# meringlab/FlashWeave.jl

Measured on AMD Instinct MI355X. Metric: ci_tests_per_sec, higher is better.
Workload: dtype f64

## Files before the change

### flashweave.jl_amd/csrc/fw_devhiton.hip

```cpp
#include <algorithm>
#include <cassert>
#include <cstring>
#include <condition_variable>
#include <mutex>
#include <thread>
#include <vector>

#include "fw_internal.h"
#define MI_MAX_K FW_MAX_K_FAST
#include "fw_mi_core.h"
#include "fw_fz_core.h"
#include "fw_unrank.h"

namespace {

struct DhTgt {
    int32_t T, phase, pos, nc;
    int32_t na, ntpc, npc, wl_n;
    long long co;
    long long cand_off;
    long long wl_off, nb_off;
    int32_t nb_n, cap;
    int32_t jactive, nsp;
    int32_t cur, pad0;
// ... 2026 lines not shown
        run += dh_ceil_div(win[act[t]], seglen, inv) + (sp[act[t]] ? dh_ceil_div(win2[act[t]], seglen, inv) * sp[act[t]] : 0u);
    }
    if (tid == 0) {
        seg0[na] = (long long)ns;
        g->ns = ns;
        g->any_big = 0u;
        g->seglen = (unsigned int)seglen;
        g->launched_ranks = total;
        g->n_live_prev = n_live;
        if (n_live == 0u) g->done = 1u;
        const unsigned int r = g->rounds;
        g->ns_ring[r & 63u] = ns;
        g->rounds = r + 1u;
        if (log && r < log_cap) log[r] = make_ulonglong2(total, ((unsigned long long)n_live << 32) | ns);
    }
}

__global__ __launch_bounds__(1024) void dh_plan_kernel(int ntg, DhGlobal *__restrict__ g, const unsigned long long *__restrict__ win,
                                                       const unsigned int *__restrict__ sp, const unsigned long long *__restrict__ win2,
                                                       const int32_t *__restrict__ act_all, long long *__restrict__ seg0, DhPlanArgs PA)
{
    dh_plan_dev<1024>(ntg, g, win, sp, win2, act_all, seg0, PA);
}
__global__ __launch_bounds__(256) void dh_plan_small_kernel(int ntg, DhGlobal *__restrict__ g, const unsigned long long *__restrict__ win,
                                                            const unsigned int *__restrict__ sp, const unsigned long long *__restrict__ win2,
                                                            const int32_t *__restrict__ act_all, long long *__restrict__ seg0, DhPlanArgs PA)
{
    dh_plan_dev<256>(ntg, g, win, sp, win2, act_all, seg0, PA);
}

__global__ __launch_bounds__(256) void dh_tmat_build_kernel(const DhTgt *__restrict__ tg, int ntg, const int32_t *__restrict__ nb_idx,
                                                            const float *__restrict__ cor, int p, float *__restrict__ tmat)
{
    __shared__ int32_t s_id[4096];
    const DhTgt &x = tg[blockIdx.x];
    if (x.tm_off < 0) return;
    const int m = x.nb_n + 1;
    const int32_t *ids = nb_idx + x.nb_off;
    for (int b = threadIdx.x; b < m; b += 256) s_id[b] = b == 0 ? x.T : ids[b - 1];
    __syncthreads();
    float *M = tmat + x.tm_off;
    for (int a0 = (int)blockIdx.y * 4; a0 < m; a0 += (int)gridDim.y * 4)
        for (int b = threadIdx.x; b < m; b += 256) {
            const size_t col = (size_t)s_id[b];
            float v[4];
#pragma unroll
            for (int q = 0; q < 4; ++q) v[q] = a0 + q < m ? cor[(size_t)s_id[a0 + q] * (size_t)p + col] : 0.0f;
#pragma unroll
            for (int q = 0; q < 4; ++q)
                if (a0 + q < m) M[(size_t)(a0 + q) * m + b] = v[q];
        }
}

__device__ __forceinline__ void dh_fill_one(const unsigned int s, const DhTgt *__restrict__ tg, int ntg, DhGlobal *__restrict__ g,
                                            const long long *__restrict__ seg0, const DhArrays &A, FwSeg *__restrict__ segs, int d1,
                                            const int32_t *__restrict__ act)
{
    int lo = 0, hi = (int)g->n_act;
    while (lo < hi) {
        const int mid = (lo + hi) >> 1;
        if (seg0[mid] <= (long long)s)
            lo = mid + 1;
        else
            hi = mid;
    }
    const DhTgt &x = tg[act[(size_t)g->act_sel * ntg + lo - 1]];
    const unsigned long long seglen = g->seglen;
    unsigned long long k = (unsigned long long)((long long)s - seg0[lo - 1]);
    const int32_t *cands = x.phase == 0 ? A.cand0 + x.cand_off : A.tpc_key + x.co;
    unsigned int slot = 0;
    if (x.nsp > 0) {
        const unsigned int all = (unsigned int)(seg0[lo] - seg0[lo - 1]);
        const unsigned int n0 = x.spmode == 1 ? dh_ceil_div(x.jwin, seglen, 1.0 / (double)seglen) : all / (1u + (unsigned int)x.nsp);
        if ((unsigned int)k >= n0) {
            const unsigned int per = (all - n0) / (unsigned int)x.nsp;
            slot = 1u + ((unsigned int)k - n0) / per;
            k -= (unsigned long long)n0 + (unsigned long long)(slot - 1u) * per;
        }
    }
    const bool acc_mode = slot > 0u && x.spmode == 1;
    FwSeg sg;
    sg.X = x.T;
    sg.Y = cands[x.pos + (int)slot];
    sg.acc_off = DH_ACC_OFF(x, x.phase == 1 ? (x.cur + (int)slot) % d1 : x.cur, d1);
    sg.acc_len = x.na + (acc_mode ? 1 : 0);
    if (sg.acc_len > FW_TAB_A) g->any_big = 1u;
    sg.pad = act[(size_t)g->act_sel * ntg + lo - 1];
    const unsigned long long lo_r = acc_mode ? 0ull : x.jnext;
    sg.start = lo_r + k * seglen;
    const unsigned long long hi_r = lo_r + (slot > 0u ? x.jwin2 : x.jwin);
    sg.end = sg.start + seglen < hi_r ? sg.start + seglen : hi_r;
    const bool has_tm = A.tmat != nullptr && x.tm_off >= 0;
    sg.tm = has_tm ? (uint64_t)(A.tmat + x.tm_off) : 0ull;
    sg.tm_ids = has_tm ? (uint64_t)(A.nb_idx + x.nb_off) : 0ull;
    sg.tm_m = has_tm ? x.nb_n + 1 : 0;
    sg.pad1 = 0;
    segs[s] = sg;
}
__global__ __launch_bounds__(256) void dh_fill_kernel(const DhTgt *__restrict__ tg, int ntg, DhGlobal *__restrict__ g,
                                                      const long long *__restrict__ seg0, const DhArrays A,
                                                      FwSeg *__restrict__ segs, int d1, const int32_t *__restrict__ act)
{
    const unsigned int s = blockIdx.x * 256 + threadIdx.x;
    if (s >= g->ns) return;
    dh_fill_one(s, tg, ntg, g, seg0, A, segs, d1, act);
}


__global__ __launch_bounds__(1024) void dh_compact_kernel(const DhTgt *__restrict__ tg, int ntg, DhGlobal *__restrict__ g,
                                                          int32_t *__restrict__ act_all)
{
    __shared__ unsigned int s_wsum[16];
    const int tid = threadIdx.x, lane = tid & 63, wave = tid >> 6;
    const int na = (int)g->n_act;
    const unsigned int sel = g->act_sel;
    const int32_t *src = act_all + (size_t)sel * ntg;
    int32_t *dst = act_all + (size_t)(sel ^ 1u) * ntg;
    const int per = (na + 1023) / 1024;
    const int b = tid * per, e = (b + per) < na ? (b + per) : na;
    unsigned int local = 0u;
    for (int i = b; i < e; ++i) {
        const DhTgt &x = tg[src[i]];
        local += (x.phase != 2 || x.jactive) ? 1u : 0u;
    }
    unsigned int incl = local;
#pragma unroll
    for (int o = 1; o < 64; o <<= 1) {
        const unsigned int v = __shfl_up(incl, o);
        if (lane >= o) incl += v;
    }
    if (lane == 63) s_wsum[wave] = incl;
    __syncthreads();
    unsigned int wbase = 0u, total = 0u;
#pragma unroll
    for (int w = 0; w < 16; ++w) {
        if (w < wave) wbase += s_wsum[w];
        total += s_wsum[w];
    }
    unsigned int pos = wbase + incl - local;
    for (int i = b; i < e; ++i) {
        const int t = src[i];
        const DhTgt &x = tg[t];
        if (x.phase != 2 || x.jactive) dst[pos++] = t;
    }
    if (tid == 0) {
        g->n_act = total;
        g->act_sel = sel ^ 1u;
    }
}

__global__ __launch_bounds__(256) void dh_nz_recs_kernel(const DhTgt *__restrict__ tg, int ntg, const DhGlobal *__restrict__ g,
                                                         const int32_t *__restrict__ act, const DhArrays A, FwNzJob *__restrict__ recs,
                                                         const long long *__restrict__ arena_off)
{
    const int ci = (int)(blockIdx.x * 256u + threadIdx.x);
    if (ci >= (int)g->n_act) return;
    const int t = act[(size_t)g->act_sel * ntg + ci];
    const DhTgt &x = tg[t];
    FwNzJob *r = recs + t;
    if (x.jactive && x.jwin > 0ull && x.jnext == 0ull) {
        r->X = x.T;
        r->Y = (x.phase == 0 ? A.cand0 + x.cand_off : A.tpc_key + x.co)[x.pos];
        r->acc_off = DH_ACC_OFF(x, x.cur, 1);
        r->acc_len = x.na;
        r->m = x.na + 2;
        r->cor_off = arena_off[t];
        r->pad = 0;
    } else {
        r->pad = 1;
    }
}

__global__ __launch_bounds__(256) void dh_sched_init_kernel(DhTgt *__restrict__ tg, int nt, const int32_t *__restrict__ tgt_T,
                                                            const long long *__restrict__ nb_off, const int32_t *__restrict__ levels,
                                                            const long long *__restrict__ slot_tm, int wl_unsorted)
{
    const int i = (int)(blockIdx.x * 256u + threadIdx.x);
    if (i >= nt) return;
    DhTgt x;
    __builtin_memset(&x, 0, sizeof(x));
    const int T = tgt_T[i];
    const long long o = nb_off[T];
    const int deg = (int)(nb_off[T + 1] - o);
    x.T = T;
    x.nc = x.cap = deg;
    x.phase = (deg == 0 || (levels && levels[T] < 2)) ? 2 : 0;
    x.co = x.cand_off = x.wl_off = x.nb_off = o;
    x.nb_n = deg;
    x.wl_unsorted = wl_unsorted;
    if (slot_tm) x.tm_off = slot_tm[i];
    tg[i] = x;
}

__global__ __launch_bounds__(256) void dh_wl_append_kernel(const DhTgt *__restrict__ tg, int ntg, const int32_t *__restrict__ pc_key,
                                                           const int32_t *__restrict__ round_of, int round, int32_t *__restrict__ wl,
                                                           const long long *__restrict__ nb_off, unsigned int *__restrict__ wl_cnt)
{
    const int t = (int)(blockIdx.x * 4u + (threadIdx.x >> 6)), lane = threadIdx.x & 63;
    if (t >= ntg) return;
    const int T = tg[t].T, npc = tg[t].npc;
    const long long co = tg[t].co;
    for (int i = lane; i < npc; i += 64) {
        const int32_t u = pc_key[co + i];
        if (round_of[u] > round) wl[nb_off[u] + (long long)atomicAdd(&wl_cnt[u], 1u)] = T;
    }
}

__global__ __launch_bounds__(256) void dh_iota_kernel(int32_t *__restrict__ act, int n)
{
    const int i = (int)(blockIdx.x * 256u + threadIdx.x);
    if (i < n) act[i] = i;
}

__global__ __launch_bounds__(256) void dh_fz_round_begin_kernel(DhTgt *__restrict__ tg, int ntg, const unsigned int *__restrict__ wl_cnt,
                                                                int32_t *__restrict__ wl, DhGlobal *__restrict__ g, long long *__restrict__ seg0,
                                                                int32_t *__restrict__ act, unsigned int *__restrict__ wl_max)
{
    __shared__ int32_t s_w[4096];
    const int t = (int)blockIdx.x, tid = (int)threadIdx.x;
    if (t >= ntg) return;
    DhTgt &x = tg[t];
    const int n = (int)wl_cnt[x.T];
    if (n > 1 && n <= 4096) {
        int32_t *w = wl + x.wl_off;
        for (int i = tid; i < n; i += 256) s_w[i] = w[i];
        __syncthreads();
        for (int i = tid; i < n; i += 256) {
            const int32_t e = s_w[i];
            int r = 0;
            for (int j = 0; j < n; ++j) r += s_w[j] < e;
            w[r] = e;
        }
    }
    if (tid == 0) {
        x.wl_n = n;
        x.wl_unsorted = n > 4096;
        act[t] = t;
        seg0[t] = 0;
        if (n > 0) atomicMax(wl_max, (unsigned int)n);
    }
    if (t == 0) {
        unsigned int *gw = (unsigned int *)g;
        for (int i = tid; i < (int)(sizeof(DhGlobal) / 4); i += 256) gw[i] = 0u;
        __syncthreads();
        if (tid == 0) {
            g->n_act = (unsigned int)ntg;
            seg0[ntg] = 0;
        }
    }
}

__global__ __launch_bounds__(256) void dh_sched_pack_kernel(const DhTgt *__restrict__ tg, int nt, const int32_t *__restrict__ pc_key,
                                                         const double *__restrict__ pc_stat, const double *__restrict__ pc_p,
                                                         int32_t *__restrict__ o_t, int32_t *__restrict__ o_u, double *__restrict__ o_s,
                                                         double *__restrict__ o_p, unsigned long long *__restrict__ tot, double *__restrict__ alg)
{
    const int t = (int)(blockIdx.x * 4u + (threadIdx.x >> 6)), lane = threadIdx.x & 63;
    if (t >= nt) return;
    const DhTgt &x = tg[t];
    const int npc = x.npc;
    unsigned long long base = 0ull;
    if (lane == 0) {
        if (npc > 0) base = atomicAdd(&tot[0], (unsigned long long)npc);
        if (x.c_ref) atomicAdd(&tot[1], x.c_ref);
        if (x.c_calls) atomicAdd(&tot[2], x.c_calls);
        if (x.c_eval) atomicAdd(&tot[3], x.c_eval);
        if (x.phase != 2) atomicAdd(&tot[4], 1ull);
        if (x.c_alg != 0.0) atomicAdd(alg, x.c_alg);
    }
    base = mi_rfl64(base);
    for (int i = lane; i < npc; i += 64) {
        o_t[base + i] = x.T;
        o_u[base + i] = pc_key[x.co + i];
        o_s[base + i] = pc_stat[x.co + i];
        o_p[base + i] = pc_p[x.co + i];
    }
}

}


static std::mutex dh_cnt_mu;

struct DhArena {
    char *base = nullptr;
    size_t used = 0;
    template <class T>
    T *take(size_t count, size_t extra_bytes = 0)
    {
        T *q = base ? (T *)(base + used) : nullptr;
        used += (sizeof(T) * count + extra_bytes + 255) & ~(size_t)255;
        return q;
    }
};
template <class Bufs, class Sizes>
static int dh_arena_reserve(fw_ctx *c, FwDevBuf &b, Bufs (*layout)(DhArena &, const Sizes &), const Sizes &z, Bufs *out)
{
    DhArena sizing;
    layout(sizing, z);
    if (int rc = fw_dev_reserve(c, b, sizing.used)) return rc;
    DhArena a{(char *)b.ptr};
    *out = layout(a, z);
    assert(a.used == sizing.used);
    return FW_OK;
}

struct DhEvents {
    hipStream_t st;
    std::vector<hipEvent_t> ev, ev_end;
    bool ok = true;
    DhEvents(hipStream_t s, int n_timing, int n_end) : st(s), ev((size_t)n_timing, nullptr), ev_end((size_t)n_end, nullptr)
    {
        for (hipEvent_t &e : ev) ok = ok && hipEventCreate(&e) == hipSuccess;
        for (hipEvent_t &e : ev_end) ok = ok && hipEventCreateWithFlags(&e, hipEventDisableTiming) == hipSuccess;
    }
    ~DhEvents()
    {
        (void)hipStreamSynchronize(st);
        for (hipEvent_t &e : ev)
            if (e) (void)hipEventDestroy(e);
        for (hipEvent_t &e : ev_end)
            if (e) (void)hipEventDestroy(e);
    }
};

static DhParams dh_make_params(fw_ctx *c, int ntg, int spec_depth, int spec0_depth)
{
    DhParams P{};
// ... 266 lines not shown
    int32_t *bacc;
    FwNzJob *nzrecs;
    long long *nzaoff;
    float *nzarena;
    DhLevel0 nb;
};
static DhRunBufs dh_run_layout(DhArena &a, const DhRunSizes &z)
{
    DhRunBufs b{};
    b.tg = a.take<DhTgt>(z.ntg);
    b.s = dh_scratch_layout(a, z.ntg, z.max_ns, z.tm_floats);
    b.cand0 = a.take<int32_t>(z.tot, 4);
    b.lists = dh_lists_layout(a, z.tot, z.d1, z.n_wl);
    if (z.log) b.log = a.take<ulonglong2>(DH_LOG_CAP);
    if (z.per_target) {
        b.mq = a.take<MiQueue>(1);
        b.boards = a.take<MiBoard>(MI_BOARD_CAP);
        b.mres = a.take<FwSegOut>(MI_REC_CAP);
        b.bacc = a.take<int32_t>(MI_BACC_CAP);
    }
    if (z.nzk) {
        b.nzrecs = a.take<FwNzJob>(z.ntg);
        b.nzaoff = a.take<long long>(z.ntg);
        b.nzarena = a.take<float>(z.nz_arena, 4);
    }
    if (z.own_nb) {
        b.nb.off = a.take<long long>(z.p + 1);
        b.nb.idx = a.take<int32_t>(z.nnz, 4);
        b.nb.stat = a.take<double>(z.nnz, 8);
        b.nb.p = a.take<double>(z.nnz, 8);
    }
    return b;
}

struct DhRun {
    fw_ctx *c;
    int chain, ntg;
    hipStream_t st;
    bool trace_host;
    DhPolicy y;
    bool use_devc;
    std::vector<DhTgt> tg;
    std::vector<int32_t> cand0, wl;
    std::vector<long long> nz_aoff;
    size_t tot = 0, tm_floats = 0, nz_arena = 0;
    int max_cap = 0, max_wl = 0;
    unsigned max_ns = 0;
    DhRunBufs D{};
    DhGlobal *hg = nullptr;
    DhArrays A{};
    DhParams P{};
    double timed_s = 0.0;
    long timed_n = 0, launches_n = 0;
    std::vector<float> log_ms;
    unsigned max_a_seen = 0;
    unsigned max_ab_seen = 0;
    bool dev_wl = false;
};

static long long dh_tm_off(const fw_ctx *c, const DhPolicy &y, int deg, size_t &tm_floats)
{
    const bool tm_on = c->P.kind == FW_FZ && c->P.max_k <= 5 && c->d_cor != nullptr && y.tm_min > 0;
    const size_t m = (size_t)deg + 1;
    if (!tm_on || deg < y.tm_min || m > 4096 || tm_floats + m * m > (size_t)1 << 32) return -1;
    const long long off = (long long)tm_floats;
    tm_floats += m * m;
    return off;
}
static unsigned dh_max_ns(const DhPolicy &y, int ntg) { return y.seg_target + (unsigned)ntg * (unsigned)(1 + DH_MAX_SPEC) + 256u; }

static void dh_build_targets(DhRun &R, const std::vector<FwDhTarget> &in)
{
    const fw_ctx *c = R.c;
    const int ntg = R.ntg;
    R.use_devc = in[0].nc_dev >= 0 && c->d_cand != nullptr;
    R.tg.resize((size_t)ntg);
    long long co = 0, wo = 0;
    for (int t = 0; t < ntg; ++t) {
        DhTgt x{};
        x.T = in[t].T;
        x.nc = R.use_devc ? in[t].nc_dev : (int32_t)in[t].cands.size();
        x.cap = x.nc;
        x.cand_off = R.use_devc ? c->nb_off[in[t].T] : co;
        x.phase = x.nc == 0 ? 2 : 0;
        x.co = co;
        x.wl_off = wo;
        x.wl_n = in[t].wl_n;
        x.nb_off = c->nb_off[x.T];
        x.nb_n = (int32_t)(c->nb_off[x.T + 1] - c->nb_off[x.T]);
        if (!R.use_devc) R.cand0.insert(R.cand0.end(), in[t].cands.begin(), in[t].cands.end());
        if (in[t].wl_n) R.wl.insert(R.wl.end(), in[t].wl, in[t].wl + in[t].wl_n);
        co += x.nc;
        wo += in[t].wl_n;
        R.max_cap = std::max(R.max_cap, x.nc);
        R.max_wl = std::max(R.max_wl, (int)in[t].wl_n);
        R.tg[t] = x;
    }
    R.tot = (size_t)co;
    for (int t = 0; t < ntg; ++t) R.tg[t].tm_off = dh_tm_off(c, R.y, R.tg[t].nb_n, R.tm_floats);
    if (R.y.nzk) {
        R.nz_aoff.resize((size_t)ntg);
        for (int t = 0; t < ntg; ++t) {
            R.nz_aoff[t] = (long long)R.nz_arena;
            const size_t mt = (size_t)(R.wl.empty() ? 1 : 2) * (size_t)R.tg[t].nc + 2;
            R.nz_arena += mt * mt;
        }
// ... 286 lines not shown
{
    const std::vector<DhTgt> &tg = R.tg;
    const int chain = R.chain;
    unsigned long long mx_ref = 0, mx_calls = 0, tot_ref = 0, tot_calls = 0;
    int t_ref = -1, t_calls = -1;
    for (const DhTgt &x : tg) {
        tot_ref += x.c_ref;
        tot_calls += x.c_calls;
        if (x.c_ref > mx_ref) mx_ref = x.c_ref, t_ref = x.T;
        if (x.c_calls > mx_calls) mx_calls = x.c_calls, t_calls = x.T;
    }
    fprintf(stderr, "[fw] chain %d: tests %llu jobs %llu; most tests in one target %llu (T=%d), most jobs in one target %llu (T=%d)\n",
            chain, tot_ref, tot_calls, mx_ref, t_ref, mx_calls, t_calls);
    unsigned long long ev_all = 0, ev_short = 0;
    int na_max = 0;
    for (const DhTgt &x : tg) {
        ev_all += x.c_eval;
        ev_short += x.c_eval_short;
        na_max = std::max(na_max, x.na_max);
    }
    fprintf(stderr, "[fw] chain %d: executed tests %llu, of them in jobs with at most %d accepted variables %llu; longest accepted list %d\n",
            chain, ev_all, (int)FW_HK_A, ev_short, na_max);
    if (R.y.per_target) {
        unsigned int t0 = ~0u;
        for (const DhTgt &x : tg) t0 = std::min(t0, x.r_first0);
        std::vector<const DhTgt *> by_end;
        for (const DhTgt &x : tg) by_end.push_back(&x);
        std::sort(by_end.begin(), by_end.end(), [&](const DhTgt *a, const DhTgt *b) { return a->r_more0 - t0 > b->r_more0 - t0; });
        for (size_t i = 0; i < by_end.size() && i < 6; ++i) {
            const DhTgt *w = by_end[i];
            fprintf(stderr, "[fw]   finished at %.2f ms (taken at %.2f): T=%d, %d candidates, %d in PC, %llu jobs, %llu tests (%llu executed); "
                            "sequential prefixes %.2f ms, board phases %.2f ms (%llu jobs went to a board; %llu team rounds)\n",
                    1e-5 * (w->r_more0 - t0), 1e-5 * (w->r_first0 - t0), w->T, w->cap, w->npc, w->c_calls, w->c_ref, w->c_eval,
                    1e-5 * w->r_first1, 1e-5 * w->r_more1, w->c_eval_short & 0xffffffffull, w->c_eval_short >> 32);
        }
    } else {
        const DhTgt *w = &tg[0];
        for (const DhTgt &x : tg)
            if (x.r_first0 + x.r_more0 + x.r_first1 + x.r_more1 > w->r_first0 + w->r_more0 + w->r_first1 + w->r_more1) w = &x;
        fprintf(stderr, "[fw] chain %d: longest-busy target T=%d: %d candidates, %d in TPC, %d in PC, %llu jobs; rounds: interleaving first windows %u, later windows %u; elimination first %u, later %u\n",
                chain, w->T, w->cap, w->ntpc, w->npc, w->c_calls, w->r_first0, w->r_more0, w->r_first1, w->r_more1);
    }
    fprintf(stderr, "[fw] chain %d: longest accepted list %u, accepted + whitelisted to come %u (most whitelisted neighbours of one target %d)\n",
            chain, R.max_a_seen, R.max_ab_seen, R.max_wl);
    fprintf(stderr, "[fw] device rounds chain %d: %d targets, set-up %.2f ms, rounds %.2f ms, results %.2f ms\n", chain, R.ntg,
            1e3 * t_setup, 1e3 * t_rounds, 1e3 * t_results);
}

static void dh_count_run(const DhRun &R, long extra_kernels)
{
    fw_ctx *c = R.c;
    std::lock_guard<std::mutex> lk(dh_cnt_mu);
    if (R.timed_n > 0) c->cnt.t_dev_subsets_s += R.timed_s * (double)R.launches_n / (double)R.timed_n;
    c->cnt.subsets_launches += R.launches_n;
    c->cnt.kernel_launches += (R.y.per_target ? R.launches_n : (R.y.nzk ? 7 : 4) * R.launches_n) + extra_kernels;
}

int fwi_devhiton_run(fw_ctx *c, const std::vector<FwDhTarget> &in, std::vector<FwDhResult> &out, FwDhFlat &flat, int chain)
{
    const int ntg = (int)in.size();
    out.assign((size_t)ntg, FwDhResult{});
    if (ntg == 0) return FW_OK;
    static const bool trace_host = fw_trace_host();
    const double th0 = fwi_now_s();
    if (chain > 0 && !c->dh_stream[chain]) FW_HIP(c, hipStreamCreateWithFlags(&c->dh_stream[chain], hipStreamNonBlocking));
    DhRun R{c, chain, ntg, chain == 0 ? c->pb[0].stream : c->dh_stream[chain], trace_host, dh_policy(c, ntg)};
    dh_build_targets(R, in);
    int rc;
    if ((rc = dh_upload(R))) return rc;
    DhEvents E(R.st, 2 * 2 * DH_BATCH, 2);
    if (!E.ok) return fw_fail(c, FW_ERR_DEVICE, "device HITON: hipEventCreate failed");
    const double th1 = fwi_now_s();
    rc = R.y.per_target ? dh_run_persistent(R, E) : DhRounds(R, E).run();
    dh_count_run(R, 0);
    if (rc) return rc;
    const double th2 = fwi_now_s();
    if ((rc = dh_download(R, out, flat))) return rc;
    if (trace_host) dh_trace_run(R, th1 - th0, th2 - th1, fwi_now_s() - th2);
    std::lock_guard<std::mutex> lk(dh_cnt_mu);
    for (const DhTgt &x : R.tg) {
        c->cnt.cond_tests_ref += (int64_t)x.c_ref;
        c->cnt.subsets_calls += (int64_t)x.c_calls;
        c->cnt.cond_tests_evaluated += (int64_t)x.c_eval;
        c->cnt.alg_bytes_subsets += x.c_alg;
    }
    return FW_OK;
}


struct DhSchedPlan {
    int nt, R, nrounds;
    std::vector<int32_t> round_of;
    DhSchedPlan(const int32_t *sched, int nt_, int R_, int p) : nt(nt_), R(R_ <= 0 || R_ > nt_ ? nt_ : R_), nrounds((nt + R - 1) / R), round_of((size_t)p, 0x7fffffff)
    {
        for (int i = 0; i < nt; ++i) round_of[sched[i]] = i / R;
    }
    int first(int r) const { return r * R; }
    int count(int r) const { return std::min(nt, r * R + R) - r * R; }
};

struct DhSchedState {
    DhTgt *tg;
    int32_t *round_of;
    unsigned int *wl_cnt;
    DhLists lists;
    int32_t *ot, *ou;
    double *os, *op;
    unsigned long long *tot;
};
static DhSchedState dh_sched_state_layout(DhArena &a, size_t nt, size_t p, size_t nnz, size_t acc_d1)
{
    DhSchedState b{};
    b.tg = a.take<DhTgt>(nt);
    b.round_of = a.take<int32_t>(p);
    b.wl_cnt = a.take<unsigned int>(p);
    b.lists = dh_lists_layout(a, nnz, acc_d1, nnz);
    b.ot = a.take<int32_t>(nnz, 4);
    b.ou = a.take<int32_t>(nnz, 4);
    b.os = a.take<double>(nnz, 8);
    b.op = a.take<double>(nnz, 8);
    b.tot = a.take<unsigned long long>(8);
    return b;
}

static int dh_sched_begin(fw_ctx *c, hipStream_t st, const DhSchedState &S, const DhSchedPlan &pl, const int32_t *d_T, const int32_t *levels,
                          const long long *slot_tm, int wl_unsorted)
{
    const size_t p = pl.round_of.size();
    FW_HIP(c, hipMemsetAsync(S.tot, 0, 64, st));
    FW_HIP(c, hipMemsetAsync(S.wl_cnt, 0, 4 * p, st));
    FW_HIP(c, hipMemcpyAsync(S.round_of, pl.round_of.data(), 4 * p, hipMemcpyHostToDevice, st));
    hipLaunchKernelGGL(dh_sched_init_kernel, dim3((unsigned)((pl.nt + 255) / 256)), dim3(256), 0, st, S.tg, pl.nt, d_T, (const long long *)c->d_nb_off, levels,
                       slot_tm, wl_unsorted);
    FW_HIP(c, hipGetLastError());
    return FW_OK;
}

static void dh_sched_append(fw_ctx *c, hipStream_t st, const DhSchedState &S, const DhTgt *tg, int ntg, int round)
{
    hipLaunchKernelGGL(dh_wl_append_kernel, dim3((unsigned)((ntg + 3) / 4)), dim3(256), 0, st, tg, ntg, (const int32_t *)S.lists.pc_key,
                       (const int32_t *)S.round_of, round, S.lists.wl, (const long long *)c->d_nb_off, S.wl_cnt);
}

static int dh_sched_pack(fw_ctx *c, hipStream_t st, const DhSchedState &S, int nt)
{
    hipLaunchKernelGGL(dh_sched_pack_kernel, dim3((unsigned)((nt + 3) / 4)), dim3(256), 0, st, (const DhTgt *)S.tg, nt, (const int32_t *)S.lists.pc_key,
                       (const double *)S.lists.pc_stat, (const double *)S.lists.pc_p, S.ot, S.ou, S.os, S.op, S.tot, (double *)(S.tot + 5));
    FW_HIP(c, hipGetLastError());
    return FW_OK;
}
static int dh_sched_totals(fw_ctx *c, hipStream_t st, const DhSchedState &S, unsigned long long (&htot)[8])
{
    FW_HIP(c, hipMemcpyAsync(htot, S.tot, 64, hipMemcpyDeviceToHost, st));
    FW_HIP(c, hipStreamSynchronize(st));
    return FW_OK;
}
static int dh_sched_finish(fw_ctx *c, hipStream_t st, const DhSchedState &S, const unsigned long long (&htot)[8], size_t nnz, FwDirected &all)
{
    if (htot[4]) return fw_fail(c, FW_ERR_DEVICE, "device schedule: %llu targets did not finish", htot[4]);
    const size_t nres = (size_t)htot[0], at0 = all.size();
    if (nres > nnz) return fw_fail(c, FW_ERR_DEVICE, "device schedule: %zu result entries for %zu level-0 entries", nres, nnz);
    all.resize(at0 + nres);
    if (nres) {
        FW_HIP(c, hipMemcpyAsync(all.t.data() + at0, S.ot, 4 * nres, hipMemcpyDeviceToHost, st));
        FW_HIP(c, hipMemcpyAsync(all.u.data() + at0, S.ou, 4 * nres, hipMemcpyDeviceToHost, st));
        FW_HIP(c, hipMemcpyAsync(all.s.data() + at0, S.os, 8 * nres, hipMemcpyDeviceToHost, st));
        FW_HIP(c, hipMemcpyAsync(all.p.data() + at0, S.op, 8 * nres, hipMemcpyDeviceToHost, st));
        FW_HIP(c, hipStreamSynchronize(st));
    }
    c->cnt.cond_tests_ref += (int64_t)htot[1];
    c->cnt.subsets_calls += (int64_t)htot[2];
    c->cnt.cond_tests_evaluated += (int64_t)htot[3];
    double alg;
    memcpy(&alg, &htot[5], sizeof(double));
    c->cnt.alg_bytes_subsets += alg;
    return FW_OK;
}


struct DhSchedSizes {
    size_t nt, p, nnz, nrounds;
};
struct DhSchedBufs {
    DhSchedState S;
    int32_t *sched, *order;
    MiQueue *mq;
    MiBoard *boards;
    FwSegOut *mres;
    int32_t *bacc;
};
static DhSchedBufs dh_sched_layout(DhArena &a, const DhSchedSizes &z)
{
    DhSchedBufs b{};
    b.S = dh_sched_state_layout(a, z.nt, z.p, z.nnz, 1);
    b.sched = a.take<int32_t>(z.nt);
    b.order = a.take<int32_t>(z.nt);
    b.mq = a.take<MiQueue>(z.nrounds);
    b.boards = a.take<MiBoard>(MI_BOARD_CAP);
    b.mres = a.take<FwSegOut>(MI_REC_CAP);
// ... 62 lines not shown
}


struct DhFzChainSizes {
    size_t ntg, max_ns, tm_floats;
};
struct DhFzSizes {
    size_t nt, p, nnz, d1, nslots;
    int K;
    DhFzChainSizes ch[FW_DH_MAX_CHAINS];
};
struct DhFzBufs {
    DhSchedState S;
    int32_t *slot_T;
    long long *slot_tm;
    unsigned int *wl_max;
    DhRoundScratch ch[FW_DH_MAX_CHAINS];
};
static DhFzBufs dh_fz_layout(DhArena &a, const DhFzSizes &z)
{
    DhFzBufs b{};
    b.S = dh_sched_state_layout(a, z.nt, z.p, z.nnz, z.d1);
    b.slot_T = a.take<int32_t>(z.nt);
    b.slot_tm = a.take<long long>(z.nt);
    b.wl_max = a.take<unsigned int>(z.nslots);
    for (int q = 0; q < z.K; ++q) b.ch[q] = dh_scratch_layout(a, z.ch[q].ntg, z.ch[q].max_ns, z.ch[q].tm_floats);
    return b;
}

struct DhFzBarrier {
    std::mutex m;
    std::condition_variable cv;
    int n, waiting = 0, rc = FW_OK;
    unsigned gen = 0;
    explicit DhFzBarrier(int k) : n(k) {}
    int arrive(int my_rc)
    {
        std::unique_lock<std::mutex> lk(m);
        if (my_rc && !rc) rc = my_rc;
        const unsigned g = gen;
        if (++waiting == n) {
            waiting = 0;
            ++gen;
            cv.notify_all();
        } else {
            cv.wait(lk, [&] { return gen != g; });
        }
        return rc;
    }
};

struct DhFzSlot {
    int base = 0, ntg = 0, max_cap = 0;
    unsigned max_ns = 0;
    size_t tm_floats = 0;
};

int fwi_devhiton_fz_schedule(fw_ctx *c, const int32_t *sched, int nt, int R, bool feed_forward, FwDirected &all)
{
    if (nt == 0) return FW_OK;
    if (!c->d_cand || !c->d_nb_idx || !c->d_nb_off) return fw_fail(c, FW_ERR_STATE, "device schedule: the level-0 lists are not on the device");
    static const bool trace_host = fw_trace_host();
    const double th0 = fwi_now_s();
    const int p = c->P.p;
    const size_t nnz = (size_t)c->nb_off[p];
    const DhSchedPlan pl(sched, nt, R, p);
    const int nrounds = pl.nrounds;
    int K = 1;
    for (int r = 0; r < nrounds; ++r) K = std::max(K, fwi_chain_count(c, (size_t)pl.count(r)));
    std::vector<DhFzSlot> slots((size_t)nrounds * (size_t)K);
    std::vector<int32_t> slot_T((size_t)nt);
    std::vector<long long> slot_tm((size_t)nt);
    DhFzSizes z{(size_t)nt, (size_t)p, nnz, 0, (size_t)nrounds * (size_t)K, K, {}};
    {
        std::vector<int> chain_of;
        std::vector<size_t> chain_idx;
        for (int r = 0; r < nrounds; ++r) {
            const int r0 = pl.first(r), n = pl.count(r);
            const int Kr = fwi_chain_count(c, (size_t)n);
            fwi_deal_chains((size_t)n, Kr, chain_of, chain_idx);
            DhFzSlot *s = &slots[(size_t)r * (size_t)K];
            for (int i = 0; i < n; ++i) ++s[chain_of[i]].ntg;
            for (int q = 0, base = r0; q < K; ++q) {
                s[q].base = base;
                base += s[q].ntg;
            }
            for (int i = 0; i < n; ++i) slot_T[(size_t)s[chain_of[i]].base + chain_idx[i]] = sched[r0 + i];
            for (int q = 0; q < K; ++q) {
                if (s[q].ntg == 0) continue;
                const DhPolicy y = dh_policy(c, s[q].ntg);
                z.d1 = (size_t)y.spec_depth + 1;
                for (int t = 0; t < s[q].ntg; ++t) {
                    const int T = slot_T[(size_t)(s[q].base + t)];
                    const int deg = (int)(c->nb_off[T + 1] - c->nb_off[T]);
                    s[q].max_cap = std::max(s[q].max_cap, deg);
                    slot_tm[(size_t)(s[q].base + t)] = dh_tm_off(c, y, deg, s[q].tm_floats);
                }
                s[q].max_ns = dh_max_ns(y, s[q].ntg);
                z.ch[q].ntg = std::max(z.ch[q].ntg, (size_t)s[q].ntg);
                z.ch[q].max_ns = std::max(z.ch[q].max_ns, (size_t)s[q].max_ns);
                z.ch[q].tm_floats = std::max(z.ch[q].tm_floats, s[q].tm_floats);
            }
        }
    }
    DhFzBufs D;
    if (int rc = dh_arena_reserve(c, c->d_dh[0], dh_fz_layout, z, &D)) return rc;
    hipStream_t sts[FW_DH_MAX_CHAINS];
    for (int q = 0; q < K; ++q) {
        if (q > 0 && !c->dh_stream[q]) FW_HIP(c, hipStreamCreateWithFlags(&c->dh_stream[q], hipStreamNonBlocking));
        sts[q] = q == 0 ? c->pb[0].stream : c->dh_stream[q];
        if (int rc = fw_pin_reserve(c, c->h_dh[q], 4096)) return rc;
    }
    static_assert(2 * sizeof(DhGlobal) <= 3072, "the pinned page holds two batch records and, at byte 3072, the whitelist word");
    hipStream_t st = sts[0];
    DhEvents X(st, 0, 3 * K);
    if (!X.ok) return fw_fail(c, FW_ERR_DEVICE, "device schedule: hipEventCreate failed");
    const DhArrays A = dh_arrays(c, c->d_cand, D.S.lists, DhLevel0{});
    FW_HIP(c, hipMemsetAsync(D.wl_max, 0, 4 * z.nslots, st));
    FW_HIP(c, hipMemcpyAsync(D.slot_T, slot_T.data(), 4 * (size_t)nt, hipMemcpyHostToDevice, st));
    FW_HIP(c, hipMemcpyAsync(D.slot_tm, slot_tm.data(), 8 * (size_t)nt, hipMemcpyHostToDevice, st));
    if (int rc = dh_sched_begin(c, st, D.S, pl, D.slot_T, nullptr, D.slot_tm, 0)) return rc;
    for (int q = 1; q < K; ++q) {
        FW_HIP(c, hipEventRecord(X.ev_end[(size_t)q * 3], st));
        FW_HIP(c, hipStreamWaitEvent(sts[q], X.ev_end[(size_t)q * 3], 0));
    }
    const double th1 = fwi_now_s();
    DhFzBarrier bar(K);
    std::vector<double> t_start((size_t)nrounds, 0.0);
    auto chain_round = [&](int q, int r, DhEvents &E) -> int {
        const DhFzSlot &s = slots[(size_t)r * (size_t)K + (size_t)q];
        hipStream_t sq = sts[q];
        if (r > 0)
            for (int o = 0; o < K; ++o)
                if (o != q) FW_HIP(c, hipStreamWaitEvent(sq, X.ev_end[(size_t)o * 3 + (size_t)((r - 1) & 1)], 0));
        if (q == 0) t_start[(size_t)r] = fwi_now_s() - th0;
        DhRun Rn{c, q, s.ntg, sq, trace_host, dh_policy(c, s.ntg)};
        Rn.use_devc = true;
        Rn.dev_wl = true;
        Rn.max_cap = s.max_cap;
        Rn.max_ns = s.max_ns;
        Rn.tm_floats = s.tm_floats;
        Rn.D.tg = D.S.tg + s.base;
        Rn.D.s = D.ch[q];
        if (!s.tm_floats) Rn.D.s.tmat = nullptr;
        const DhRoundScratch &cb = Rn.D.s;
        Rn.A = A;
        Rn.A.tmat = cb.tmat;
        Rn.hg = (DhGlobal *)c->h_dh[q].ptr;
        memset(Rn.hg, 0, 2 * sizeof(DhGlobal));
        unsigned int *h_wl_max = (unsigned int *)((char *)c->h_dh[q].ptr + 3072);
        unsigned int *d_wl_max = D.wl_max + (size_t)r * (size_t)K + (size_t)q;
        hipLaunchKernelGGL(dh_fz_round_begin_kernel, dim3((unsigned)s.ntg), dim3(256), 0, sq, Rn.D.tg, s.ntg, (const unsigned int *)D.S.wl_cnt, D.S.lists.wl,
                           cb.g, cb.seg0, cb.act, d_wl_max);
        FW_HIP(c, hipGetLastError());
        if (feed_forward && r > 0) {
            FW_HIP(c, hipMemcpyAsync(h_wl_max, d_wl_max, sizeof(unsigned int), hipMemcpyDeviceToHost, sq));
            FW_HIP(c, hipEventRecord(X.ev_end[(size_t)q * 3 + 2], sq));
        }
        if (cb.tmat) {
            hipLaunchKernelGGL(dh_tmat_build_kernel, dim3((unsigned)s.ntg, 8u), dim3(256), 0, sq, (const DhTgt *)Rn.D.tg, s.ntg, A.nb_idx,
                               (const float *)c->d_cor, p, cb.tmat);
            FW_HIP(c, hipGetLastError());
        }
        Rn.P = dh_make_params(c, s.ntg, Rn.y.spec_depth, Rn.y.spec0_depth);
        if (feed_forward && r > 0) {
            FW_HIP(c, hipEventSynchronize(X.ev_end[(size_t)q * 3 + 2]));
            Rn.max_wl = (int)*h_wl_max;
        }
        int rc = DhRounds(Rn, E).run();
        const bool append = !rc && feed_forward && r + 1 < nrounds;
        dh_count_run(Rn, 1 + (cb.tmat ? 1 : 0) + (append ? 1 : 0));
        if (rc) return rc;
        if (append) {
            dh_sched_append(c, sq, D.S, Rn.D.tg, s.ntg, r);
            FW_HIP(c, hipGetLastError());
        }
        return FW_OK;
    };
    auto chain_body = [&](int q) {
        DhEvents E(sts[q], 2 * 2 * DH_BATCH, 2);
        int rc = E.ok ? FW_OK : fw_fail(c, FW_ERR_DEVICE, "device schedule: hipEventCreate failed");
        for (int r = 0; r < nrounds; ++r) {
            if (!rc && slots[(size_t)r * (size_t)K + (size_t)q].ntg > 0) rc = chain_round(q, r, E);
            if (!rc && hipEventRecord(X.ev_end[(size_t)q * 3 + (size_t)(r & 1)], sts[q]) != hipSuccess)
                rc = fw_fail(c, FW_ERR_DEVICE, "device schedule: hipEventRecord failed");
            if ((rc = bar.arrive(rc))) break;
        }
    };
    {
        std::vector<std::thread> th;
        for (int q = 1; q < K; ++q)
            th.emplace_back([&, q] {
                (void)hipSetDevice(c->P.device);
                chain_body(q);
            });
        chain_body(0);
        for (std::thread &t : th) t.join();
    }
    if (bar.rc) return bar.rc;
    const double th2 = fwi_now_s();
    if (int rc = dh_sched_pack(c, st, D.S, nt)) return rc;
    unsigned long long htot[8] = {0, 0, 0, 0, 0, 0, 0, 0};
    if (int rc = dh_sched_totals(c, st, D.S, htot)) return rc;
    if (int rc = dh_sched_finish(c, st, D.S, htot, nnz, all)) return rc;
    c->cnt.kernel_launches += 2;
    if (trace_host) {
        fprintf(stderr, "[fw] fz device schedule: %d targets in %d rounds on %d chains, set-up %.2f ms, rounds %.2f ms, results %.2f ms; rounds start at", nt,
                nrounds, K, 1e3 * (th1 - th0), 1e3 * (th2 - th1), 1e3 * (fwi_now_s() - th2));
        for (int r = 0; r < nrounds; ++r) fprintf(stderr, " %.2f", 1e3 * t_start[(size_t)r]);
        fprintf(stderr, " ms\n");
    }
    return FW_OK;
}
```

### flashweave.jl_amd/csrc/fw_knobs.h

```cpp
#pragma once
#include <cstdlib>

#define FW_KNOB_LIST(X)                                                                                                                                                   \
                                                                    \
    X(FW_HOST_HITON, "1: HITON-PC through the host job pool instead of the device rounds; default 0")                                                                     \
    X(FW_HOST_BH, "1: Benjamini-Hochberg and neighbour lists on the host instead of fw_bh.hip; default 0")                                                                \
    X(FW_DEV_MIN_TARGETS, "fewest targets of a round that take the device path; default 64 (fz, fz_nz) / 256 (discrete)")                                                 \
    X(FW_NZ_DEV, "0: fz_nz rounds through the host pool; default on")                                                                                                     \
    X(FW_MI_SCHED, "0: discrete kinds as one launch per round with the host in between instead of the device schedule; default on")                                       \
    X(FW_FZ_SCHED, "0: fz feed-forward rounds one by one with the host in between instead of the device schedule; default on")                                            \
    X(FW_MI_ROUNDS, "non-zero: discrete kinds as level-synchronous rounds over the segment kernels instead of the persistent kernel; default 0")                          \
    X(FW_DH_CHAINS, "concurrent chains of device rounds (fz), clamped to 1..4; default 2")                                                                                \
    X(FW_DH_CHAINS_DISC, "the same for the discrete kinds under FW_MI_ROUNDS, clamped to 1..4; default 2")                                                                \
    X(FW_DH_CHAIN_MIN, "targets per chain below which a round stays on one chain (positive); default 48")                                                                 \
    X(FW_DH_HEAVY_PCT, "percent of the heaviest targets that get chain 0 to themselves in small rounds; default 0 (off)")                                                 \
    X(FW_DH_HEAVY_BELOW, "... only in rounds of at most this many targets; default 512")                                                                                  \
    X(FW_FZS_GRAM, "0: streamed-column tests without the Gram-matrix kernel; default on")                                                                                 \
    X(FW_NO_HK, "set: generic size-4/5 kernel for every job instead of the level-2 table kernel; default unset")                                                          \
    X(FW_NO_TAB, "set: in-lane caching kernel for every job instead of the table kernel; default unset")                                                                  \
    X(FW_ZC_OUT, "0: segment results staged through device memory instead of written to pinned host memory; default on")                                                  \
    X(FW_L0_MFMA, "discrete level 0 on the matrix cores: 0 never, 2 wherever defined; default 1 (mi_nz from 1 024 variables on)")                                         \
    X(FW_MI_ROWK, "row-count form of the discrete test core, 99: popcount form only; default 2")                                                                          \
    X(FW_MI_ROW4, "0: one subset per wavefront step, 2: four per step up to MI4_N samples; default 1 (four up to 2 048 samples)")                                         \
                                                                                                                 \
    X(FW_WINDOW_GROWTH, "2..64: fixed growth factor of a job's evaluation window; default 0 (by launch size, see fw_window_growth)")                                      \
    X(FW_SMALL_LAUNCH, "ranks below which a launch counts as small and windows grow x256; default 4194304")                                                               \
    X(FW_W0_BIG, "first window of a job with 64 accepted variables or more; default 16384 (device rounds, fz max_k <= 3: 32768, see dh_make_params)")                     \
    X(FW_W0_SMALL, "first window of a smaller job in the device rounds (positive, fz only); default per kind / max_k, see dh_make_params")                                \
    X(FW_SEG_TARGET, "workgroups per launch the segment length aims for (positive); default per kind / max_k, see dh_policy and pool_round")                              \
    X(FW_SPEC_DEPTH, "candidates the host pool tests ahead per target; default 8")                                                                                        \
    X(FW_SPEC_TARGETS, "... in rounds of at most this many targets; default 512")                                                                                         \
                                                                      \
    X(FW_ELIM_FULL, "0: elimination jobs start with a first window like interleaving jobs instead of the full enumeration; default 1")                                    \
    X(FW_DH_GROWTH, "window growth factor of a job (positive); default 4")                                                                                                \
    X(FW_DH_GROWTH_SMALL, "... after a launch of fewer than FW_SMALL_LAUNCH ranks (positive); default 256")                                                               \
    X(FW_DH_GROWTH_BUSY, "... with more than FW_DH_BUSY_JOBS live jobs (positive); default 4")                                                                            \
    X(FW_DH_BUSY_JOBS, "live jobs from which a round counts as busy (positive); default 2048")                                                                            \
    X(FW_DH_SPEC, "elimination look-ahead: members tested ahead per target, clamped to 0..DH_MAX_SPEC; default 4 (exact elimination: DH_SPEC_EXACT)")                     \
    X(FW_DH_SPEC_BELOW, "... only after a launch of fewer ranks than this (positive); default 30000000 (max_k <= 3, 256 targets or more) / 12000000")                     \
    X(FW_DH_SPEC0, "interleaving look-ahead: candidates tested ahead per target, clamped to 0..DH_MAX_SPEC; default 2")                                                   \
    X(FW_DH_SPEC0_BELOW, "... only after a launch of fewer ranks than this (positive); default 12000000")                                                                 \
    X(FW_DH_SPEC0_JOBS, "... and of fewer jobs than this (positive); default 4096")                                                                                       \
    X(FW_DH_SPEC0_LIGHT, "deeper interleaving look-ahead after light launches, at least FW_DH_SPEC0; default FW_DH_SPEC0")                                                \
    X(FW_DH_SPEC0_LIGHT_BELOW, "ranks below which a launch counts as light (positive); default 400000")                                                                   \
    X(FW_DH_SPEC1, "look-ahead behind a candidate about to be accepted (fz), clamped to 0..DH_MAX_SPEC; default 2")                                                       \
    X(FW_SEG_A, "launches of fewer ranks than this use a third of FW_SEG_TARGET (fz); default 8000000")                                                                   \
    X(FW_SEG_B, "... fewer than this, two thirds; default 12000000")                                                                                                      \
    X(FW_SEG_GRID, "cap on the striding workgroups of the segment kernel (positive); default 2048 (fz, max_k <= 3) / FW_SEG_TARGET + 512")                                \
    X(FW_FZ_TMAT, "smallest degree of a target that gets a local correlation matrix, 0: none; default 16 (max_k > 3: 1)")                                                 \
    X(FW_DH_BATCH, "rounds per batch (positive, at most 16); default 4 up to 1 024 targets, else 16")                                                                     \
    X(FW_DH_TIME_EVERY, "one segment launch in this many is timed with events (positive); default 4")                                                                     \
    X(FW_DH_HP, "1: step / compact / plan / fill kernels on a high-priority stream; default off")                                                                         \
    X(FW_DH_PLAN_SMALL, "0: the 1 024-thread plan kernel instead of the 256-thread one; default 1")                                                                       \
                                                                                                 \
    X(FW_MI_SEQ, "tests a job runs before it opens a board (positive); default 48")                                                                                       \
    X(FW_MI_SEQ_HEAVY, "... for a job of a heavy target (FW_MI_HEAVY); default FW_MI_SEQ")                                                                                \
    X(FW_MI_SEQ_TAIL, "... once the target list is exhausted (tail of a launch); default 4")                                                                              \
    X(FW_MI_HEAVY, "candidates from which a target never works on other targets' boards, 0: off; default 48")                                                             \
    X(FW_MI_WIN0, "first window of a board (positive); default 128")                                                                                                      \
    X(FW_MI_WIN0_TAIL, "... in the tail of a launch (at least 1); default 1024")                                                                                          \
    X(FW_MI_CHUNK_DIV, "ranks per record of a board: its window over this (positive); default 256")                                                                       \
    X(FW_MI_CHUNK_MIN, "... at least this (positive); default 8")                                                                                                         \
    X(FW_MI_CHUNK_MAX, "... at most this (positive); default 64")                                                                                                         \
    X(FW_MI_CHUNK_TAIL, "... at least this in the tail of a launch (at least 1); default FW_MI_CHUNK_MIN")                                                                \
    X(FW_MI_HELP_JOBS, "0: idle wavefronts do not help on other targets' boards; default 1")                                                                              \
    X(FW_MI_ELIM_MIN, "elimination jobs of more ranks than this open a board for the whole enumeration at once, 0: off; default 64")                                      \
    X(FW_MI_AHEAD, "0: no first tests of up to four interleaving candidates in one step (mi_first4); default 1")                                                          \
    X(FW_MI_TEAM_MIN, "candidates from which a target is run by a whole workgroup, 0: none; default 96")                                                                  \
    X(FW_MI_TEAM_MAX, "most such targets per launch; default 192")                                                                                                        \
    X(FW_MI_TEAM_STEPS, "lock-step rounds of a team job before its enumeration goes to a board; default 2")                                                               \
    X(FW_MI_TEAM_TAIL, "non-zero: team targets publish tail-mode boards from the start; default 0")                                                                       \
    X(FW_MI_WG_PER_CU, "workgroups of the persistent kernel per compute unit (positive); default 1")                                                                      \
                                                                                              \
    X(FW_TRACE_HOST, "set: host-side phase times, per-chain test counts and list lengths on stderr; default unset")                                                       \
    X(FW_TRACE_ROUNDS, "file: one line per round of the host pool; default unset")                                                                                        \
    X(FW_TRACE_JOBS, "file: one line per finished job of the host pool; default unset")                                                                                   \
    X(FW_DH_LOG, "file: one line per planned launch of the device rounds (profiles/README.md); default unset")                                                            \
    X(FW_NZ_TRACE, "set: shape of every fz_nz sub-matrix launch on stderr; default unset")                                                                                \
    X(FW_L0_VERBOSE, "set: pair / candidate counts and phase cycles of the discrete level 0 on stderr; default unset")                                                    \
    X(FW_MI_PROF, "set: shader cycles per phase of the discrete batch tests; default unset")                                                                              \
    X(FW_L0_DBG, "discrete level-0 ablations, bits 1 no epilogue, 2 no loads, 4 no popcounts, 8 no exact pass; default 0")                                                \
    X(FW_FZ_DBG, "Fisher-z kernel ablation flags (fz_dbg_flags); default 0")

namespace knob {
enum Id {
#define X(name, doc) name,
    FW_KNOB_LIST(X)
#undef X
        COUNT
};
}

inline const char *fw_knob_str(knob::Id k)
{
    static const char *const names[knob::COUNT] = {
#define X(name, doc) #name,
        FW_KNOB_LIST(X)
#undef X
    };
    const char *on = getenv("FW_KNOBS");
    return (on && on[0] == '1') ? getenv(names[k]) : nullptr;
// ... 27 lines not shown
```

Baseline: 83.80 billion.

## Run low-degree targets end-to-end in one workgroup and batch pack-kernel atomics

Adds a prepass kernel that gives each low-degree target its own workgroup, which loops advance, segment test and merge/commit until the target is done. This takes those targets out of the batched multi-kernel round machinery, which is skipped entirely when every target is light. The sched pack kernel now uses one thread per target, with a wave prefix sum and reductions, so there is one set of atomics per wave instead of per target. The light path only runs for f32 FZ with max_k <= 3, so it may be off for an f64 workload. Its serial per-target loop can also leave the GPU underused when targets vary in size.

Result: faster. 86.71 billion (median of 6 runs) (+3.5%).

```diff
diff --git a/flashweave.jl_amd/csrc/fw_devhiton.hip b/flashweave.jl_amd/csrc/fw_devhiton.hip
--- a/flashweave.jl_amd/csrc/fw_devhiton.hip
+++ b/flashweave.jl_amd/csrc/fw_devhiton.hip
@@ -2102,6 +2102,25 @@
         }
 }
 
+__device__ __forceinline__ FwSeg dh_seg_record(const DhTgt &x, const DhArrays &A, int32_t Y, long long acc_off, int acc_len, int32_t pad,
+                                               unsigned long long start, unsigned long long end)
+{
+    FwSeg sg;
+    sg.X = x.T;
+    sg.Y = Y;
+    sg.acc_off = acc_off;
+    sg.acc_len = acc_len;
+    sg.pad = pad;
+    sg.start = start;
+    sg.end = end;
+    const bool has_tm = A.tmat != nullptr && x.tm_off >= 0;
+    sg.tm = has_tm ? (uint64_t)(A.tmat + x.tm_off) : 0ull;
+    sg.tm_ids = has_tm ? (uint64_t)(A.nb_idx + x.nb_off) : 0ull;
+    sg.tm_m = has_tm ? x.nb_n + 1 : 0;
+    sg.pad1 = 0;
+    return sg;
+}
+
 __device__ __forceinline__ void dh_fill_one(const unsigned int s, const DhTgt *__restrict__ tg, int ntg, DhGlobal *__restrict__ g,
                                             const long long *__restrict__ seg0, const DhArrays &A, FwSeg *__restrict__ segs, int d1,
                                             const int32_t *__restrict__ act)
@@ -2129,23 +2148,13 @@
         }
     }
     const bool acc_mode = slot > 0u && x.spmode == 1;
-    FwSeg sg;
-    sg.X = x.T;
-    sg.Y = cands[x.pos + (int)slot];
-    sg.acc_off = DH_ACC_OFF(x, x.phase == 1 ? (x.cur + (int)slot) % d1 : x.cur, d1);
-    sg.acc_len = x.na + (acc_mode ? 1 : 0);
-    if (sg.acc_len > FW_TAB_A) g->any_big = 1u;
-    sg.pad = act[(size_t)g->act_sel * ntg + lo - 1];
+    const int acc_len = x.na + (acc_mode ? 1 : 0);
+    if (acc_len > FW_TAB_A) g->any_big = 1u;
     const unsigned long long lo_r = acc_mode ? 0ull : x.jnext;
-    sg.start = lo_r + k * seglen;
+    const unsigned long long start = lo_r + k * seglen;
     const unsigned long long hi_r = lo_r + (slot > 0u ? x.jwin2 : x.jwin);
-    sg.end = sg.start + seglen < hi_r ? sg.start + seglen : hi_r;
-    const bool has_tm = A.tmat != nullptr && x.tm_off >= 0;
-    sg.tm = has_tm ? (uint64_t)(A.tmat + x.tm_off) : 0ull;
-    sg.tm_ids = has_tm ? (uint64_t)(A.nb_idx + x.nb_off) : 0ull;
-    sg.tm_m = has_tm ? x.nb_n + 1 : 0;
-    sg.pad1 = 0;
-    segs[s] = sg;
+    segs[s] = dh_seg_record(x, A, cands[x.pos + (int)slot], DH_ACC_OFF(x, x.phase == 1 ? (x.cur + (int)slot) % d1 : x.cur, d1), acc_len,
+                            act[(size_t)g->act_sel * ntg + lo - 1], start, start + seglen < hi_r ? start + seglen : hi_r);
 }
 __global__ __launch_bounds__(256) void dh_fill_kernel(const DhTgt *__restrict__ tg, int ntg, DhGlobal *__restrict__ g,
                                                       const long long *__restrict__ seg0, const DhArrays A,
@@ -2221,6 +2230,69 @@
     }
 }
 
+__host__ __device__ inline bool dh_is_light(int deg, int cap, int light_deg) { return light_deg > 0 && deg <= light_deg && cap <= light_deg; }
+
+__shared__ DhTgt dh_lt_x;
+__shared__ FwSeg dh_lt_seg;
+__shared__ int dh_lt_go;
+
+__global__ __launch_bounds__(256, 4) void dh_fz_light_kernel(DhTgt *__restrict__ tg, int ntg, int light_deg, const DhArrays A,
+                                                             FwSegOut *__restrict__ so, const DhParams P, const float *__restrict__ cor, int p,
+                                                             double zscale, const double *__restrict__ thr)
+{
+    const int t = (int)blockIdx.x, tid = (int)threadIdx.x, lane = tid & 63;
+    if (t >= ntg || !dh_is_light(tg[t].nb_n, tg[t].cap, light_deg)) return;
+    const int d1 = P.spec_depth + 1;
+    const int job_max = 2 * tg[t].cap;
+    for (int job = 0;; ++job) {
+        if (tid < 64) {
+            DhTgt x = job == 0 ? tg[t] : dh_lt_x;
+            if (job > 0) {
+                const DhMerge M = dh_merge(so, (long long)t, 1, lane);
+                const double r_stat = M.stop ? M.stat : (M.p != -2.0 ? M.stat : 0.0);
+                const double r_p = M.stop ? M.p : (M.p < 0.0 ? 0.0 : M.p);
+                (x.phase == 0 ? x.r_first0 : x.r_first1) += 1u;
+                x.c_ref += M.stop ? M.nt : x.jN;
+                x.c_calls += 1ull;
+                x.c_eval += M.ev;
+                x.c_eval_short += x.na <= FW_HK_A ? M.ev : 0ull;
+                x.na_max = x.na > x.na_max ? x.na : x.na_max;
+                x.c_alg += dh_alg_bytes(x.na, M.ev, P.max_k, P.disc_bytes_per_col);
+                dh_commit(x, A, lane, d1, r_stat, r_p, M.stop ? M.pow : 1, P.alpha, P.elim_mode != 0);
+            }
+            bool go = x.phase != 2 && dh_advance(x, A, lane, d1, P.elim_mode == 2);
+            go = go && job < job_max && x.na <= FW_TAB_A;
+            if (go) x.jN = dh_enum_size(x.na, P.max_k, P.max_tests);
+            if (lane == 0) {
+                dh_lt_x = x;
+                dh_lt_go = go ? 1 : 0;
+                if (go)
+                    dh_lt_seg = dh_seg_record(x, A, (x.phase == 0 ? A.cand0 + x.cand_off : A.tpc_key + x.co)[x.pos], DH_ACC_OFF(x, x.cur, d1),
+                                              x.na, t, 0ull, x.jN);
+            }
+        }
+        __builtin_amdgcn_fence(__ATOMIC_SEQ_CST, "workgroup");
+        __syncthreads();
+        if (!dh_lt_go) break;
+        FwSeg sg = dh_lt_seg;
+        sg.X = __builtin_amdgcn_readfirstlane(sg.X);
+        sg.Y = __builtin_amdgcn_readfirstlane(sg.Y);
+        sg.acc_off = (int64_t)mi_rfl64((unsigned long long)sg.acc_off);
+        sg.acc_len = __builtin_amdgcn_readfirstlane(sg.acc_len);
+        sg.pad = __builtin_amdgcn_readfirstlane(sg.pad);
+        sg.start = mi_rfl64(sg.start);
+        sg.end = mi_rfl64(sg.end);
+        sg.tm = mi_rfl64(sg.tm);
+        sg.tm_ids = mi_rfl64(sg.tm_ids);
+        sg.tm_m = __builtin_amdgcn_readfirstlane(sg.tm_m);
+        fz_seg_body<false, false, true>(cor, p, sg, A.acc + sg.acc_off, false, so + t, P.max_k, P.alpha, zscale, P.max_tests, thr,
+                                        (const FwNzJob *)nullptr, 0ll);
+        __builtin_amdgcn_fence(__ATOMIC_SEQ_CST, "workgroup");
+        __syncthreads();
+    }
+    if (tid == 0) tg[t] = dh_lt_x;
+}
+
 __global__ __launch_bounds__(256) void dh_sched_init_kernel(DhTgt *__restrict__ tg, int nt, const int32_t *__restrict__ tgt_T,
                                                             const long long *__restrict__ nb_off, const int32_t *__restrict__ levels,
                                                             const long long *__restrict__ slot_tm, int wl_unsorted)
@@ -2305,25 +2377,56 @@
                                                          int32_t *__restrict__ o_t, int32_t *__restrict__ o_u, double *__restrict__ o_s,
                                                          double *__restrict__ o_p, unsigned long long *__restrict__ tot, double *__restrict__ alg)
 {
-    const int t = (int)(blockIdx.x * 4u + (threadIdx.x >> 6)), lane = threadIdx.x & 63;
-    if (t >= nt) return;
-    const DhTgt &x = tg[t];
-    const int npc = x.npc;
-    unsigned long long base = 0ull;
-    if (lane == 0) {
-        if (npc > 0) base = atomicAdd(&tot[0], (unsigned long long)npc);
-        if (x.c_ref) atomicAdd(&tot[1], x.c_ref);
-        if (x.c_calls) atomicAdd(&tot[2], x.c_calls);
-        if (x.c_eval) atomicAdd(&tot[3], x.c_eval);
-        if (x.phase != 2) atomicAdd(&tot[4], 1ull);
-        if (x.c_alg != 0.0) atomicAdd(alg, x.c_alg);
-    }
-    base = mi_rfl64(base);
-    for (int i = lane; i < npc; i += 64) {
-        o_t[base + i] = x.T;
-        o_u[base + i] = pc_key[x.co + i];
-        o_s[base + i] = pc_stat[x.co + i];
-        o_p[base + i] = pc_p[x.co + i];
+    __shared__ unsigned long long s_base[256];
+    const int tid = (int)threadIdx.x, lane = tid & 63, t = (int)blockIdx.x * 256 + tid;
+    unsigned long long npc = 0ull, ref = 0ull, calls = 0ull, ev = 0ull, unfinished = 0ull;
+    double al = 0.0;
+    if (t < nt) {
+        const DhTgt &x = tg[t];
+        npc = (unsigned long long)x.npc;
+        ref = x.c_ref;
+        calls = x.c_calls;
+        ev = x.c_eval;
+        unfinished = x.phase != 2 ? 1ull : 0ull;
+        al = x.c_alg;
+    }
+    unsigned long long incl = npc;
+#pragma unroll
+    for (int o = 1; o < 64; o <<= 1) {
+        const unsigned long long v = __shfl_up(incl, o);
+        if (lane >= o) incl += v;
+    }
+#pragma unroll
+    for (int o = 32; o > 0; o >>= 1) {
+        ref += __shfl_xor(ref, o);
+        calls += __shfl_xor(calls, o);
+        ev += __shfl_xor(ev, o);
+        unfinished += __shfl_xor(unfinished, o);
+        al += __shfl_xor(al, o);
+    }
+    unsigned long long wbase = 0ull;
+    if (lane == 63) {
+        if (incl) wbase = atomicAdd(&tot[0], incl);
+        if (ref) atomicAdd(&tot[1], ref);
+        if (calls) atomicAdd(&tot[2], calls);
+        if (ev) atomicAdd(&tot[3], ev);
+        if (unfinished) atomicAdd(&tot[4], unfinished);
+        if (al != 0.0) atomicAdd(alg, al);
+    }
+    s_base[tid] = __shfl(wbase, 63) + incl - npc;
+    __syncthreads();
+    for (int j = 0; j < 64; ++j) {
+        const int u = tid - lane + j, tu = (int)blockIdx.x * 256 + u;
+        if (tu >= nt) break;
+        const DhTgt &x = tg[tu];
+        const unsigned long long base = s_base[u];
+        const int n = x.npc;
+        for (int i = lane; i < n; i += 64) {
+            o_t[base + i] = x.T;
+            o_u[base + i] = pc_key[x.co + i];
+            o_s[base + i] = pc_stat[x.co + i];
+            o_p[base + i] = pc_p[x.co + i];
+        }
     }
 }
 
@@ -2696,6 +2799,7 @@
     DhParams P{};
     double timed_s = 0.0;
     long timed_n = 0, launches_n = 0;
+    long light_n = 0;
     std::vector<float> log_ms;
     unsigned max_a_seen = 0;
     unsigned max_ab_seen = 0;
@@ -3088,8 +3192,27 @@
     fw_ctx *c = R.c;
     std::lock_guard<std::mutex> lk(dh_cnt_mu);
     if (R.timed_n > 0) c->cnt.t_dev_subsets_s += R.timed_s * (double)R.launches_n / (double)R.timed_n;
-    c->cnt.subsets_launches += R.launches_n;
-    c->cnt.kernel_launches += (R.y.per_target ? R.launches_n : (R.y.nzk ? 7 : 4) * R.launches_n) + extra_kernels;
+    c->cnt.subsets_launches += R.launches_n + R.light_n;
+    c->cnt.kernel_launches += (R.y.per_target ? R.launches_n : (R.y.nzk ? 7 : 4) * R.launches_n) + R.light_n + extra_kernels;
+}
+
+static int dh_light_deg(const fw_ctx *c, const DhPolicy &y)
+{
+    if (c->P.kind != FW_FZ || c->f64 || !c->d_cor || c->P.max_k < 1 || c->P.max_k > 3 || c->d_rej_run || y.per_target) return 0;
+    return std::min(std::max(fw_knob_int(knob::FW_DH_LIGHT_DEG, 32), 0), FW_TAB_A / 2);
+}
+
+static int dh_light_prepass(DhRun &R, int light_deg, int n_light)
+{
+    if (n_light == 0) return FW_OK;
+    fw_ctx *c = R.c;
+    double zscale = 0.0;
+    if (int rc = fwi_fz_thresholds(c, R.st, &zscale)) return rc;
+    hipLaunchKernelGGL(dh_fz_light_kernel, dim3((unsigned)R.ntg), dim3(256), 0, R.st, R.D.tg, R.ntg, light_deg, R.A, R.D.s.so, R.P,
+                       (const float *)c->d_cor, c->P.p, zscale, (const double *)c->d_thr);
+    FW_HIP(c, hipGetLastError());
+    R.light_n = 1;
+    return FW_OK;
 }
 
 int fwi_devhiton_run(fw_ctx *c, const std::vector<FwDhTarget> &in, std::vector<FwDhResult> &out, FwDhFlat &flat, int chain)
@@ -3107,7 +3230,15 @@
     DhEvents E(R.st, 2 * 2 * DH_BATCH, 2);
     if (!E.ok) return fw_fail(c, FW_ERR_DEVICE, "device HITON: hipEventCreate failed");
     const double th1 = fwi_now_s();
-    rc = R.y.per_target ? dh_run_persistent(R, E) : DhRounds(R, E).run();
+    if (R.y.per_target) {
+        rc = dh_run_persistent(R, E);
+    } else {
+        const int light_deg = dh_light_deg(c, R.y);
+        int n_light = 0;
+        for (const DhTgt &x : R.tg) n_light += dh_is_light(x.nb_n, x.cap, light_deg) ? 1 : 0;
+        rc = dh_light_prepass(R, light_deg, n_light);
+        if (!rc && n_light < ntg) rc = DhRounds(R, E).run();
+    }
     dh_count_run(R, 0);
     if (rc) return rc;
     const double th2 = fwi_now_s();
@@ -3180,7 +3311,7 @@
 
 static int dh_sched_pack(fw_ctx *c, hipStream_t st, const DhSchedState &S, int nt)
 {
-    hipLaunchKernelGGL(dh_sched_pack_kernel, dim3((unsigned)((nt + 3) / 4)), dim3(256), 0, st, (const DhTgt *)S.tg, nt, (const int32_t *)S.lists.pc_key,
+    hipLaunchKernelGGL(dh_sched_pack_kernel, dim3((unsigned)((nt + 255) / 256)), dim3(256), 0, st, (const DhTgt *)S.tg, nt, (const int32_t *)S.lists.pc_key,
                        (const double *)S.lists.pc_stat, (const double *)S.lists.pc_p, S.ot, S.ou, S.os, S.op, S.tot, (double *)(S.tot + 5));
     FW_HIP(c, hipGetLastError());
     return FW_OK;
@@ -3349,6 +3480,7 @@
 
 struct DhFzSlot {
     int base = 0, ntg = 0, max_cap = 0;
+    int n_light = 0;
     unsigned max_ns = 0;
     size_t tm_floats = 0;
 };
@@ -3386,11 +3518,13 @@
             for (int q = 0; q < K; ++q) {
                 if (s[q].ntg == 0) continue;
                 const DhPolicy y = dh_policy(c, s[q].ntg);
+                const int light_deg = dh_light_deg(c, y);
                 z.d1 = (size_t)y.spec_depth + 1;
                 for (int t = 0; t < s[q].ntg; ++t) {
                     const int T = slot_T[(size_t)(s[q].base + t)];
                     const int deg = (int)(c->nb_off[T + 1] - c->nb_off[T]);
                     s[q].max_cap = std::max(s[q].max_cap, deg);
+                    s[q].n_light += dh_is_light(deg, deg, light_deg) ? 1 : 0;
                     slot_tm[(size_t)(s[q].base + t)] = dh_tm_off(c, y, deg, s[q].tm_floats);
                 }
                 s[q].max_ns = dh_max_ns(y, s[q].ntg);
@@ -3450,7 +3584,8 @@
         hipLaunchKernelGGL(dh_fz_round_begin_kernel, dim3((unsigned)s.ntg), dim3(256), 0, sq, Rn.D.tg, s.ntg, (const unsigned int *)D.S.wl_cnt, D.S.lists.wl,
                            cb.g, cb.seg0, cb.act, d_wl_max);
         FW_HIP(c, hipGetLastError());
-        if (feed_forward && r > 0) {
+        const bool rounds = s.n_light < s.ntg;
+        if (rounds && feed_forward && r > 0) {
             FW_HIP(c, hipMemcpyAsync(h_wl_max, d_wl_max, sizeof(unsigned int), hipMemcpyDeviceToHost, sq));
             FW_HIP(c, hipEventRecord(X.ev_end[(size_t)q * 3 + 2], sq));
         }
@@ -3460,11 +3595,12 @@
             FW_HIP(c, hipGetLastError());
         }
         Rn.P = dh_make_params(c, s.ntg, Rn.y.spec_depth, Rn.y.spec0_depth);
-        if (feed_forward && r > 0) {
+        int rc = dh_light_prepass(Rn, dh_light_deg(c, Rn.y), s.n_light);
+        if (!rc && rounds && feed_forward && r > 0) {
             FW_HIP(c, hipEventSynchronize(X.ev_end[(size_t)q * 3 + 2]));
             Rn.max_wl = (int)*h_wl_max;
         }
-        int rc = DhRounds(Rn, E).run();
+        if (!rc && rounds) rc = DhRounds(Rn, E).run();
         const bool append = !rc && feed_forward && r + 1 < nrounds;
         dh_count_run(Rn, 1 + (cb.tmat ? 1 : 0) + (append ? 1 : 0));
         if (rc) return rc;
diff --git a/flashweave.jl_amd/csrc/fw_knobs.h b/flashweave.jl_amd/csrc/fw_knobs.h
--- a/flashweave.jl_amd/csrc/fw_knobs.h
+++ b/flashweave.jl_amd/csrc/fw_knobs.h
@@ -47,6 +47,7 @@
     X(FW_SEG_A, "launches of fewer ranks than this use a third of FW_SEG_TARGET (fz); default 8000000")                                                                   \
     X(FW_SEG_B, "... fewer than this, two thirds; default 12000000")                                                                                                      \
     X(FW_SEG_GRID, "cap on the striding workgroups of the segment kernel (positive); default 2048 (fz, max_k <= 3) / FW_SEG_TARGET + 512")                                \
+    X(FW_DH_LIGHT_DEG, "largest level-0 degree of a target that one workgroup runs from start to end (fz, max_k <= 3), clamped to FW_TAB_A / 2, 0: off; default 32")      \
     X(FW_FZ_TMAT, "smallest degree of a target that gets a local correlation matrix, 0: none; default 16 (max_k > 3: 1)")                                                 \
     X(FW_DH_BATCH, "rounds per batch (positive, at most 16); default 4 up to 1 024 targets, else 16")                                                                     \
     X(FW_DH_TIME_EVERY, "one segment launch in this many is timed with events (positive); default 4")                                                                     \
```
